# nagyrajmund/st-gcn

Measured on AMD Instinct MI355X. Metric: skeleton clips/sec (fwd+bwd), synthetic (N,3,300,18); 1/2/4/8-GPU scaling, higher is better.
Workload: dtype fp32; 1 GPU; cfg2 Kinetics-skeleton shape: 10-block ST-GCN stack fwd+bwd+CE+Adam, V=18, T=300, K=1 (uni), 400 classes; per_gpu_batch=128, global_batch=128, seq_len=300, parallelism=dp1

## Files before the change

### st-gcn_amd/csrc/internal.h

```cpp
#pragma once
#include <hip/hip_runtime.h>
#include <stdint.h>

#include <type_traits>

namespace stgcn {

struct Dropout {
  uint64_t seed = 0;
  uint32_t thresh = 0;
  float scale = 1.f;
  const uint64_t *seed_dev = nullptr;
};

constexpr uint64_t kDropGolden = 0x9E3779B97F4A7C15ull;

__host__ __device__ inline uint64_t mix64(uint64_t z) {
  z = (z ^ (z >> 30)) * 0xBF58476D1CE4E5B9ull;
  z = (z ^ (z >> 27)) * 0x94D049BB133111EBull;
  return z ^ (z >> 31);
}

__host__ __device__ inline bool dropout_keep(const Dropout &d, uint64_t e) {
  return (uint32_t)(mix64(d.seed + e * kDropGolden) >> 32) >= d.thresh;
// ... 58 lines not shown
  PrevBn prev;
  double *sd, *sdn;
  float *dA;
  float *dA_part;
  int wpk_ready;
  int bna;
  int w4;
};

struct WgradParams {
  const float *P, *Q;
  float *slab;
  int64_t p_bstride, q_bstride;
  int R, C, NQ, s_in, off;
  int M;
  int T_src;
  int V, FT;
  int n_mtiles, n_rtiles, n_jtiles, S, N;
  int CT;
  int bf16;
  int p_bf16, q_bf16;
  int f16x2;
  const unsigned *amax_p, *amax_q;
  BnRef q_bn;
  int x3_mr;
};

hipError_t launch_conv_gemm(const ConvGemmParams &p, hipStream_t s);
hipError_t launch_absmax(const float *x, int64_t n, unsigned *amax, hipStream_t s);
size_t fold_fwd_scratch_floats(int R, int C, int V);
size_t fold_bwd_scratch_floats(int R, int C);
size_t fold_sdz_scratch_doubles(int R, int C, int V);
size_t fold_dwc_floats(int R, int C);
hipError_t launch_fold_w(const float *Wt, const float *W, int R, int C, float *Wc, float *scratch,
                         hipStream_t s);
hipError_t launch_fold_fwd(const float *Wt, const float *W, const float *bt, const float *bZ, int R,
                           int C, int V, int T, int To, int st, float *Wc, double *bq, float *BT,
                           float *scratch, hipStream_t s);
hipError_t launch_fold_prep_bwd(const float *Wt, const float *W, int R, int C, float *scratch,
                                hipStream_t s);
hipError_t launch_fold_tq(const double *cs, int nz, int R, int T, int To, int V, int st,
                          double *Tq, double *tqT, hipStream_t s);
double *fold_sdz_tq_slot(double *scratch, int R, int C);
hipError_t launch_fold_sdz(double *scratch, const float *Wt, const float *Wc, const double *Tq,
                           int R, int C, int V, double *SdZ, double *SdH, hipStream_t s,
                           bool pre = false, const double *tqT = nullptr);
hipError_t launch_fold_small_sd(const double *SdZ, const float *A, const float *bW, int R, int V,
                                float *dbW, float *dA, const double *SdH, int C, double *sd,
                                hipStream_t s);
struct FoldPrepSpec {
  const float *A, *W, *bW, *Wt, *bWt;
  int R, C, V, T, To, stride;
  float *bZ, *Wc, *BT, *fscr_f, *fscr_b;
  double *bq, *f64;
  unsigned *amax;
};
hipError_t launch_fold_prep(const FoldPrepSpec *specs, int n, hipStream_t s);
hipError_t launch_fold_grads(const float *slab, int S, const float *scratch, const float *bZ,
                             const double *Tq, int R, int C, int V, float *dwc, float *dWt,
                             float *dW, hipStream_t s);
struct Bn2Bwd {
  const float *dy = nullptr, *dy_nc = nullptr, *U = nullptr;
  BnRef bn;
  const double *sg = nullptr, *sgu = nullptr;
  float *dU = nullptr, *dUA = nullptr;
  double *sdu = nullptr, *cs = nullptr;
  int N = 0, C = 0, L = 0, V = 0;
  int training = 1;
  Dropout drop;
  int du_bf16 = 0;
  const float *dy_coef = nullptr;
  unsigned *amax = nullptr, *amaxa = nullptr;
  const float *A = nullptr;
};
int apply_cols_chunks(int N);
hipError_t launch_bn_relu_bwd_reduce(const Bn2Bwd &q, double *sg, double *sgu, hipStream_t s);
hipError_t launch_bn_relu_bwd_apply(const Bn2Bwd &q, hipStream_t s);
hipError_t launch_bn_relu_bwd_apply_cols(const Bn2Bwd &q, hipStream_t s);
hipError_t launch_bn_relu_bwd_apply_fr(const Bn2Bwd &q, hipStream_t s);
bool conv_bf16_supported(const ConvGemmParams &p);
size_t conv_bf16_lds_bytes(const ConvGemmParams &p);
hipError_t launch_conv_bf16(const ConvGemmParams &p, hipStream_t s);
bool conv_x3_supported(const ConvGemmParams &p);
constexpr int kPackJobs = 16;
struct PackJob {
  const float *w;
  void *wpk;
  int R, C, NQ, TG, nch, rows, npl;
  int64_t w_sr, w_sc, w_sq, total;
  const unsigned *amax_w;
};
PackJob conv_x3_pack_job(const ConvGemmParams &p, int npl);
size_t conv_x3_pack_bytes(const ConvGemmParams &p, int npl);
hipError_t launch_pack_jobs(const PackJob *jobs, int n, hipStream_t s);
bool conv_x3_bna_supported(const ConvGemmParams &p);
size_t conv_x3_wpk_bytes(const ConvGemmParams &p);
hipError_t launch_conv_x3(const ConvGemmParams &p, hipStream_t s);
bool conv_b1_supported(const ConvGemmParams &p);
hipError_t launch_conv_b1(const ConvGemmParams &p, hipStream_t s);
bool plan_wgrad_x3(WgradParams &w, bool f16x2);
hipError_t launch_wgrad_x3(const WgradParams &p, hipStream_t s);
bool plan_wgrad_bf16(WgradParams &w);
hipError_t launch_wgrad_bf16(const WgradParams &p, hipStream_t s);
hipError_t launch_wgrad(const WgradParams &p, hipStream_t s);
void plan_wgrad_sp(WgradParams &p);
bool wgrad_sp_applies(const WgradParams &p);
inline int wgrad_sp_kc(int CT) { return CT == 64 ? 64 : 32; }
hipError_t launch_wgrad_taps(const WgradParams &p, hipStream_t s);
int wgrad_taps_cb(const WgradParams &p);
size_t wgrad_taps_lds_bytes(const WgradParams &p);
bool wgrad_taps_supported(const WgradParams &p);
size_t conv_gemm_lds_bytes(const ConvGemmParams &p);
size_t conv_gemm_wpk_floats(const ConvGemmParams &p);
bool conv_gemm_supported(const ConvGemmParams &p);
size_t wgrad_lds_bytes(const WgradParams &p);
bool wgrad_supported(const WgradParams &p);
int wgrad_ntiles_j(int C, int NQ);

hipError_t launch_slab_reduce(const float *slab, int S, int64_t n, float *dst, int mode,
                              int R, int K, int C, hipStream_t s);

hipError_t launch_bn_stats(const float *x, int N, int C, int L, double *sum, double *sq,
                           hipStream_t s, unsigned *amax = nullptr);
hipError_t launch_bn_finalize(const double *sum, const double *sq, int C, int64_t M,
                              float eps, float momentum, int training, float *rm, float *rv,
                              float *mean_out, float *invstd_out, hipStream_t s, unsigned *zw = nullptr,
                              int nzw = 0);
hipError_t launch_bn_relu_fwd(const float *U, const BnRef &bn, float *y, int N, int C, int L,
                              double *ysum, double *ysq, Dropout drop, hipStream_t s,
                              double *yext = nullptr, unsigned *ymax = nullptr);
hipError_t launch_chain_coef(const double *sd, const double *sdn, const BnRef &bn1,
                             const double *s1, const double *s2, const double *xst, int C,
                             int64_t M, float *dg1, float *db1, float *coef, double *psum,
                             hipStream_t s);
hipError_t launch_bn_grads_out(const double *sg, const double *sgu, const double *sdu, int C,
                               float *dgamma, float *dbeta, float *dbias, hipStream_t s);
hipError_t launch_bn1_bwd_apply(float *dx, const float *x, const BnRef &bn1, const double *sd,
                                const double *sdn, const float *add, int N, int C, int L,
                                int64_t M, int training, const BnRef &pbn2, double *psum,
                                const float *pU, hipStream_t s);
hipError_t launch_relu_bwd(const float *dy, const float *y, float *dout, double *sum, int N,
                           int C, int L, float scale, hipStream_t s);

hipError_t launch_pack_w(const float *W, float *Wpk, int K, int R, int C, hipStream_t s);
hipError_t launch_bias_rv(const float *A, const float *bW, float *bias_rv, int K, int R, int V,
                          hipStream_t s);
hipError_t launch_bn_finalize_parts(const double *part, int ntiles, int C, int64_t M, float eps,
                                    float momentum, int training, float *rm, float *rv,
                                    float *mean_out, float *invstd_out, hipStream_t s,
                                    double *ys_zero = nullptr, int nw = 0);
template <class F>
inline auto dispatch_v(int V, F &&f) {
  if (V == 18) return f(std::integral_constant<int, 18>{});
  if (V == 25) return f(std::integral_constant<int, 25>{});
  return f(std::integral_constant<int, 50>{});
}

struct SpatialFwd {
  const float *x = nullptr;
  BnRef bn;
  const float *A = nullptr;
  int N = 0, C = 0, R = 0, T = 0, V = 0, K = 0, relu = 0;
  PrevBn prev;
  float *G = nullptr;
  unsigned *amax = nullptr;
  const float *W = nullptr, *biasZ = nullptr;
  void *wpk = nullptr;
// ... 46 lines not shown
```

### st-gcn_amd/csrc/kernels_fold.hip

```cpp
#include <hip/hip_runtime.h>

#include <algorithm>
#include <initializer_list>
#include <vector>

#include "device_common.h"
#include "internal.h"

#define HIP_RET(expr)                  \
  do {                                 \
    hipError_t e_ = (expr);            \
    if (e_ != hipSuccess) return e_;   \
  } while (0)

namespace stgcn {

typedef float float8v __attribute__((ext_vector_type(8)));
typedef double double4v __attribute__((ext_vector_type(4)));

__host__ __device__ inline int pad32(int x) { return (x + 31) & ~31; }

struct FoldJob {
  const float *A, *B;
  int64_t aq, am, bq, bn;
  const double *A2;
  const float *B2;
  int64_t a2q, a2m, b2n;
  void *out;
  int64_t oq, om, on;
  int o_dbl, red;
  int M, N, K, K2;
};

constexpr int kFoldJobs = 18;
struct FoldJobs {
  FoldJob j[kFoldJobs];
  int n;
  int tile0[kFoldJobs + 1];
};

template <int NG>
__device__ __forceinline__ void f32_stream(const float *pa, const float *pb, floatx4 &acc) {
  constexpr int D = NG < 4 ? NG : 4;
  float4 a[D], b[D];
#pragma unroll
  for (int d = 0; d < D; ++d) {
    a[d] = *reinterpret_cast<const float4 *>(pa + 16 * d);
    b[d] = *reinterpret_cast<const float4 *>(pb + 16 * d);
  }
  __builtin_amdgcn_sched_barrier(0);
#pragma unroll
  for (int i = 0; i < NG; ++i) {
    const int d = i % D;
    acc = __builtin_amdgcn_mfma_f32_16x16x4f32(a[d].x, b[d].x, acc, 0, 0, 0);
    acc = __builtin_amdgcn_mfma_f32_16x16x4f32(a[d].y, b[d].y, acc, 0, 0, 0);
    acc = __builtin_amdgcn_mfma_f32_16x16x4f32(a[d].z, b[d].z, acc, 0, 0, 0);
    acc = __builtin_amdgcn_mfma_f32_16x16x4f32(a[d].w, b[d].w, acc, 0, 0, 0);
    if (i + D < NG) {
      a[d] = *reinterpret_cast<const float4 *>(pa + 16 * (i + D));
      b[d] = *reinterpret_cast<const float4 *>(pb + 16 * (i + D));
    }
    __builtin_amdgcn_sched_barrier(0);
  }
}

__device__ __forceinline__ void f32_stream_any(const float *pa, const float *pb, int ng,
                                               floatx4 &acc) {
  switch (ng) {
    case 4: f32_stream<4>(pa, pb, acc); return;
    case 8: f32_stream<8>(pa, pb, acc); return;
    case 16: f32_stream<16>(pa, pb, acc); return;
    default: break;
  }
  for (int i = 0; i < ng; i += 4) {
    if (ng - i >= 4) {
      f32_stream<4>(pa + 16 * i, pb + 16 * i, acc);
    } else {
      for (int k = i; k < ng; ++k) f32_stream<1>(pa + 16 * k, pb + 16 * k, acc);
    }
  }
}

__global__ __launch_bounds__(576) void k_fold_gemm(FoldJobs js) {
  __shared__ float red[9][16 * 17];
  const int tile = blockIdx.x;
  int ji = 0;
  while (ji + 1 < js.n && tile >= js.tile0[ji + 1]) ++ji;
  const FoldJob &g = js.j[ji];
  const int t = tile - js.tile0[ji], ntn = (g.N + 15) >> 4;
  const int m0 = (t / ntn) * 16, n0 = (t % ntn) * 16;
  const int q = threadIdx.x >> 6, l = threadIdx.x & 63, r16 = l & 15, kq = l >> 4;
  floatx4 acc = {0.f, 0.f, 0.f, 0.f};
  {
    const float *pa = g.A + q * g.aq + (int64_t)(m0 + r16) * g.am + 4 * kq;
    const float *pb = g.B + q * g.bq + (int64_t)(n0 + r16) * g.bn + 4 * kq;
    f32_stream_any(pa, pb, (g.K + 15) >> 4, acc);
  }
  if (g.A2) {
    const int m = m0 + r16, n = n0 + r16;
    const bool ok_m = m < g.M, ok_n = n < g.N;
    const double *a2 = g.A2 + q * g.a2q + (int64_t)min(m, g.M - 1) * g.a2m;
    const float *b2 = g.B2 + (int64_t)min(n, g.N - 1) * g.b2n;
    for (int k0 = 0; k0 < g.K2; k0 += 4) {
      const int k = k0 + kq, kc = min(k, g.K2 - 1);
      const float x = (float)a2[kc], y = b2[kc];
      acc = __builtin_amdgcn_mfma_f32_16x16x4f32(k < g.K2 && ok_m ? x : 0.f,
                                                 k < g.K2 && ok_n ? y : 0.f, acc, 0, 0, 0);
    }
  }
  if (!g.red) {
    const int nn = n0 + r16;
#pragma unroll
    for (int r = 0; r < 4; ++r) {
      const int mm = m0 + 4 * kq + r;
      if (mm >= g.M || nn >= g.N) continue;
      const int64_t o = q * g.oq + mm * g.om + nn * g.on;
      if (g.o_dbl)
        reinterpret_cast<double *>(g.out)[o] = acc[r];
      else
        reinterpret_cast<float *>(g.out)[o] = acc[r];
    }
    return;
  }
#pragma unroll
  for (int r = 0; r < 4; ++r) red[q][(4 * kq + r) * 17 + r16] = acc[r];
  __syncthreads();
  if (threadIdx.x >= 256) return;
  const int rr = threadIdx.x >> 4, cc = threadIdx.x & 15;
  const int mm = m0 + rr, nn = n0 + cc;
  if (mm >= g.M || nn >= g.N) return;
  double sum = 0.0;
#pragma unroll
  for (int w = 0; w < 9; ++w) sum += red[w][rr * 17 + cc];
  const int64_t o = mm * g.om + nn * g.on;
  if (g.o_dbl)
    reinterpret_cast<double *>(g.out)[o] = sum;
  else
    reinterpret_cast<float *>(g.out)[o] = (float)sum;
}

static hipError_t fold_gemm_v(const FoldJob *jobs, int n, hipStream_t s) {
  for (int i0 = 0; i0 < n; i0 += kFoldJobs) {
    FoldJobs js{};
    js.n = 0;
    int tiles = 0;
    for (int i = i0; i < std::min(n, i0 + kFoldJobs); ++i) {
      const FoldJob &g = jobs[i];
      if (g.M <= 0 || g.N <= 0) return hipErrorInvalidValue;
      js.j[js.n] = g;
      js.tile0[js.n++] = tiles;
      tiles += ((g.M + 15) / 16) * ((g.N + 15) / 16);
    }
    js.tile0[js.n] = tiles;
    hipLaunchKernelGGL(k_fold_gemm, dim3(tiles), dim3(576), 0, s, js);
  }
  return hipGetLastError();
}

static hipError_t fold_gemm(std::initializer_list<FoldJob> jobs, hipStream_t s) {
  return fold_gemm_v(jobs.begin(), (int)jobs.size(), s);
}

struct TrJob {
  const void *src;
  int s_dbl, S, nq, q_inner;
  int64_t sstride, sq, so, si;
  int O, I;
  void *outQ, *outT;
  int o_dbl;
  int tiles_i;
};

constexpr int kTrJobs = 16;
struct TrJobs {
  TrJob j[kTrJobs];
  int n;
  int tile0[kTrJobs + 1];
};

__global__ __launch_bounds__(576) void k_fold_tr(TrJobs js) {
  __shared__ double tile[36 * 16 + 4];
  const int blk = blockIdx.x, tid = threadIdx.x;
  int ji = 0;
  while (ji + 1 < js.n && blk >= js.tile0[ji + 1]) ++ji;
  const TrJob &g = js.j[ji];
  const int t = blk - js.tile0[ji];
  const int nq = g.nq, OT = nq == 9 ? 4 : 36;
  const int o0 = (t / g.tiles_i) * OT, i0 = (t % g.tiles_i) * 16;
  const int Op = pad32(g.O), Ip = pad32(g.I);
  int oo, ii, q;
  if (nq == 1) {
    oo = tid >> 4; ii = tid & 15; q = 0;
  } else if (g.q_inner) {
    oo = tid / 144; const int r = tid - oo * 144; ii = r / 9; q = r - ii * 9;
  } else {
    oo = tid / 144; const int r = tid - oo * 144; q = r >> 4; ii = r & 15;
  }
  const int o = o0 + oo, i = i0 + ii;
  double v = 0.0;
  if (o < g.O && i < g.I) {
    const int64_t at = q * g.sq + o * g.so + i * g.si;
    if (g.s_dbl) {
      v = reinterpret_cast<const double *>(g.src)[at];
    } else {
      const float *p = reinterpret_cast<const float *>(g.src) + at;
      int k = 0;
      for (; k + 16 <= g.S; k += 16) {
        float a[16];
#pragma unroll
        for (int u = 0; u < 16; ++u) a[u] = p[(int64_t)(k + u) * g.sstride];
#pragma unroll
        for (int u = 0; u < 16; ++u) v += a[u];
      }
      for (; k + 4 <= g.S; k += 4) {
        const float a0 = p[k * g.sstride], a1 = p[(k + 1) * g.sstride],
                    a2 = p[(k + 2) * g.sstride], a3 = p[(k + 3) * g.sstride];
        v += a0;
        v += a1;
        v += a2;
        v += a3;
      }
      for (; k < g.S; ++k) v += p[k * g.sstride];
    }
  }
  const int slot = (q * OT + oo) * 16 + ii;
  tile[slot + slot / 16 / 8] = v;
  __syncthreads();
  if (g.outQ) {
    const int sq2 = tid / (OT * 16), a = (tid >> 4) % OT, b = tid & 15;
    const int s2 = (sq2 * OT + a) * 16 + b;
    const int64_t at = ((int64_t)sq2 * Op + o0 + a) * Ip + i0 + b;
    if (o0 + a < Op) {
      if (g.o_dbl)
        reinterpret_cast<double *>(g.outQ)[at] = tile[s2 + s2 / 16 / 8];
      else
        reinterpret_cast<float *>(g.outQ)[at] = (float)tile[s2 + s2 / 16 / 8];
    }
  }
  if (g.outT) {
    const int sq2 = tid / (OT * 16), a = (tid / OT) & 15, b = tid % OT;
    const int s2 = (sq2 * OT + b) * 16 + a;
    const int64_t at = ((int64_t)sq2 * Ip + i0 + a) * Op + o0 + b;
    if (o0 + b < Op) {
      if (g.o_dbl)
        reinterpret_cast<double *>(g.outT)[at] = tile[s2 + s2 / 16 / 8];
      else
        reinterpret_cast<float *>(g.outT)[at] = (float)tile[s2 + s2 / 16 / 8];
    }
  }
}

static TrJob tr_job(const void *src, int s_dbl, int S, int64_t sstride, int nq, int64_t sq,
                    int64_t so, int64_t si, int O, int I, float *outQ, float *outT,
                    double *outQd = nullptr, double *outTd = nullptr) {
  TrJob g{};
  g.src = src; g.s_dbl = s_dbl; g.S = S; g.sstride = sstride;
  g.nq = nq; g.sq = sq; g.so = so; g.si = si; g.q_inner = sq == 1;
  g.O = O; g.I = I; g.outQ = outQ; g.outT = outT;
  if (outQd || outTd) {
    g.o_dbl = 1;
    g.outQ = outQd;
    g.outT = outTd;
  }
  g.tiles_i = pad32(I) / 16;
  return g;
}

static hipError_t fold_tr_v(const TrJob *jobs, int n, hipStream_t s) {
  for (int i0 = 0; i0 < n; i0 += kTrJobs) {
    TrJobs js{};
    int tiles = 0;
    for (int i = i0; i < std::min(n, i0 + kTrJobs); ++i) {
      const TrJob &g = jobs[i];
      if ((g.nq != 1 && g.nq != 9) || g.O <= 0 || g.I <= 0) return hipErrorInvalidValue;
      js.j[js.n] = g;
      js.tile0[js.n++] = tiles;
      const int OT = g.nq == 9 ? 4 : 36;
      tiles += g.tiles_i * ((pad32(g.O) + OT - 1) / OT);
    }
    js.tile0[js.n] = tiles;
    hipLaunchKernelGGL(k_fold_tr, dim3(tiles), dim3(576), 0, s, js);
  }
  return hipGetLastError();
}

static hipError_t fold_tr(std::initializer_list<TrJob> jobs, hipStream_t s) {
  return fold_tr_v(jobs.begin(), (int)jobs.size(), s);
}

size_t fold_fwd_scratch_floats(int R, int C, int V) {
  const int Rp = pad32(R);
  return (size_t)Rp * (9 * Rp + pad32(C) + pad32(V));
}

static hipError_t fold_fwd_gemms(const float *Wt, const float *W, const float *bZ, int R, int C,
                                 int V, float *Wc, double *bq, float *scratch, hipStream_t s) {
  const int Rp = pad32(R), Cp = pad32(C);
  float *wtq = scratch, *wT = wtq + (size_t)9 * Rp * Rp, *bzT = wT + (size_t)Cp * Rp;
  const TrJob ja = tr_job(Wt, 0, 1, 0, 9, 1, (int64_t)R * 9, 9, R, R, wtq, nullptr);
  const TrJob jb = tr_job(W, 0, 1, 0, 1, 0, C, 1, R, C, nullptr, wT);
  if (bq)
    HIP_RET(fold_tr({ja, jb, tr_job(bZ, 0, 1, 0, 1, 0, V, 1, R, V, nullptr, bzT)}, s));
  else
    HIP_RET(fold_tr({ja, jb}, s));
  FoldJob w{};
  w.A = wtq; w.aq = (int64_t)Rp * Rp; w.am = Rp;
  w.B = wT; w.bn = Rp;
  w.out = Wc; w.oq = 1; w.om = (int64_t)C * 9; w.on = 9;
  w.M = R; w.N = C; w.K = R;
  if (!bq) return fold_gemm({w}, s);
  FoldJob b{};
  b.A = wtq; b.aq = (int64_t)Rp * Rp; b.am = Rp;
  b.B = bzT; b.bn = Rp;
  b.out = bq; b.o_dbl = 1; b.oq = (int64_t)R * V; b.om = V; b.on = 1;
  b.M = R; b.N = V; b.K = R;
  return fold_gemm({w, b}, s);
}

hipError_t launch_fold_w(const float *Wt, const float *W, int R, int C, float *Wc, float *scratch,
                         hipStream_t s) {
  return fold_fwd_gemms(Wt, W, nullptr, R, C, 0, Wc, nullptr, scratch, s);
}

__device__ __forceinline__ int fold_slot_frame(int slot, int nb0, int tb1) {
  return slot < nb0 ? slot : tb1 + slot - nb0;
}

__global__ __launch_bounds__(256) void k_fold_bias(const double *bq, const float *bt, int R, int V,
                                                   int T, int To, int st, float *BT) {
  __shared__ double bs[9 * 256], full[256];
  const int o = blockIdx.x, tid = threadIdx.x;
  for (int e = tid; e < 9 * V; e += 256) {
    const int q = e / V, v = e - q * V;
    bs[e] = bq[((int64_t)q * R + o) * V + v];
  }
  __syncthreads();
  const double b0 = bt[o];
  if (tid < V) {
    double a = b0;
#pragma unroll
    for (int q = 0; q < 9; ++q) a += bs[q * V + tid];
    full[tid] = a;
  }
  __syncthreads();
  float *dst = BT + (int64_t)o * To * V;
  for (int tv = tid; tv < To * V; tv += 256) {
    const int t = tv / V, v = tv - t * V, t0 = st * t - 4;
    double a;
    if (t0 >= 0 && t0 + 8 < T) {
      a = full[v];
    } else {
      a = b0;
      for (int q = 0; q < 9; ++q)
        if (t0 + q >= 0 && t0 + q < T) a += bs[q * V + v];
    }
    dst[tv] = (float)a;
  }
}

static hipError_t fold_bias_frames(const double *bq, const float *bt, int R, int V, int T, int To,
                                   int st, float *BT, hipStream_t s) {
  if (V > 256) return hipErrorInvalidValue;
  hipLaunchKernelGGL(k_fold_bias, dim3(R), dim3(256), 0, s, bq, bt, R, V, T, To, st, BT);
  return hipGetLastError();
}

hipError_t launch_fold_fwd(const float *Wt, const float *W, const float *bt, const float *bZ, int R,
                           int C, int V, int T, int To, int st, float *Wc, double *bq, float *BT,
                           float *scratch, hipStream_t s) {
  HIP_RET(fold_fwd_gemms(Wt, W, bZ, R, C, V, Wc, bq, scratch, s));
  return fold_bias_frames(bq, bt, R, V, T, To, st, BT, s);
}


constexpr int kTqThreads = 1024;
__global__ __launch_bounds__(kTqThreads) void k_fold_tq(const double *cs, int nz, int R, int V,
                                                        int T, int To, int st, int nb0, int tb1,
                                                        double *Tq, double *tqT) {
  __shared__ double ts[kTqThreads], bs[8 * 256];
  const int o = blockIdx.x, tid = threadIdx.x;
  const int Rp = pad32(R), Vp = pad32(V);
  if (o >= R) {
    for (int e = tid; e < 9 * Vp; e += kTqThreads) tqT[(int64_t)e * Rp + o] = 0.0;
    return;
  }
  const int PH = kTqThreads / V, ph = tid / V, v = tid - ph * V;
  const int nsl = nb0 + (To - tb1);
  const int64_t zs = (int64_t)R * To * V;
  double a = 0.0;
  if (ph < PH) {
    const int nj = nz * To;
    auto at = [&](int j) {
      const int z = j / To, t = j - z * To;
      return cs[z * zs + ((int64_t)o * To + t) * V + v];
    };
    double a0 = 0.0, a1 = 0.0, a2 = 0.0, a3 = 0.0;
    int j = ph;
    for (; j + 3 * PH < nj; j += 4 * PH) {
      const double x0 = at(j), x1 = at(j + PH), x2 = at(j + 2 * PH), x3 = at(j + 3 * PH);
      a0 += x0;
      a1 += x1;
      a2 += x2;
      a3 += x3;
    }
    for (; j < nj; j += PH) a0 += at(j);
    a = (a0 + a1) + (a2 + a3);
    for (int sl = ph; sl < nsl; sl += PH) {
      const int t = fold_slot_frame(sl, nb0, tb1);
      double b = 0.0;
      for (int z = 0; z < nz; ++z) b += cs[z * zs + ((int64_t)o * To + t) * V + v];
      bs[sl * V + v] = b;
    }
  }
  ts[tid] = a;
  __syncthreads();
  if (tqT && tid >= V && tid < Vp)
    for (int q = 0; q < 9; ++q) tqT[((int64_t)q * Vp + tid) * Rp + o] = 0.0;
  if (tid >= V) return;
  double tot = 0.0;
  for (int p = 0; p < PH; ++p) tot += ts[p * V + tid];
  for (int q = 0; q < 9; ++q) {
    double r = tot;
    for (int sl = 0; sl < nsl; ++sl) {
      const int tt = st * fold_slot_frame(sl, nb0, tb1) + q - 4;
      if (tt < 0 || tt >= T) r -= bs[sl * V + tid];
    }
    Tq[((int64_t)q * R + o) * V + tid] = r;
    if (tqT) tqT[((int64_t)q * Vp + tid) * Rp + o] = r;
  }
}

void fold_slots(int T, int To, int st, int &nb0, int &tb1) {
  nb0 = std::min(To, (4 + st - 1) / st);
  tb1 = std::max(nb0, std::min(To, (T - 4 + st - 1) / st));
}

hipError_t launch_fold_tq(const double *cs, int nz, int R, int T, int To, int V, int st,
                          double *Tq, double *tqT, hipStream_t s) {
  if (V > 256) return hipErrorInvalidValue;
  int nb0, tb1;
// ... 163 lines not shown
  } else if (Wc) {
    HIP_RET(fold_tr({jt, tr_job(Wc, 0, 1, 0, 9, 1, (int64_t)C * 9, 9, R, C, nullptr, nullptr,
                                nullptr, wcT)},
                    s));
  } else {
    HIP_RET(fold_tr({jt}, s));
  }
  Red64Jobs js{};
  Red64Job z{};
  z.A = wtT; z.aq = (int64_t)Rp * Rp; z.am = Rp;
  z.B = tqT; z.bq = (int64_t)Vp * Rp; z.bn = Rp;
  z.out = SdZ; z.om = V;
  z.M = R; z.N = V; z.K = R;
  js.j[0] = z;
  js.n = 1;
  const int tz = ((R + 15) / 16) * ((V + 15) / 16);
  js.tile0[1] = tz;
  int tiles = tz;
  if (Wc && SdH) {
    Red64Job h = z;
    h.A = wcT; h.aq = (int64_t)Cp * Rp;
    h.out = SdH;
    h.M = C;
    js.j[1] = h;
    js.n = 2;
    tiles += ((C + 15) / 16) * ((V + 15) / 16);
  }
  js.tile0[js.n] = tiles;
  hipLaunchKernelGGL(k_fold_red64, dim3(tiles), dim3(576), 0, s, js);
  return hipGetLastError();
}

__global__ __launch_bounds__(256) void k_fold_small_sd(const double *SdZ, const float *A,
                                                       const float *bW, int R, int V, float *dbW,
                                                       float *dA, const double *SdH, int C,
                                                       double *sd) {
  __shared__ double rs[256], part[256];
  const int tid = threadIdx.x;
  for (int v = tid; v < V; v += 256) {
    double ra = 0.0;
    for (int w = 0; w < V; ++w) ra += (double)A[v * V + w];
    rs[v] = ra;
  }
  __syncthreads();
  if (blockIdx.x > 0) {
    const int c = (blockIdx.x - 1) * blockDim.x + tid;
    if (c >= C) return;
    double a = 0.0;
    for (int v = 0; v < V; ++v) a += SdH[(int64_t)c * V + v] * rs[v];
    sd[c] = a;
    return;
  }
  for (int co = tid; co < R; co += 256) {
    double acc = 0.0;
    for (int v = 0; v < V; ++v) acc += SdZ[co * V + v] * rs[v];
    dbW[co] = (float)acc;
  }
  const int P = 256 / V;
  const int v = tid % V, j = tid / V;
  double acc = 0.0;
  if (j < P)
    for (int co = j; co < R; co += P) acc += (double)bW[co] * SdZ[co * V + v];
  part[tid] = acc;
  __syncthreads();
  if (tid < V) {
    double t = 0.0;
    for (int jj = 0; jj < P; ++jj) t += part[jj * V + tid];
    rs[tid] = t;
  }
  __syncthreads();
  for (int i = tid; i < V * V; i += 256) dA[i] = (float)rs[i / V];
}

hipError_t launch_fold_small_sd(const double *SdZ, const float *A, const float *bW, int R, int V,
                                float *dbW, float *dA, const double *SdH, int C, double *sd,
                                hipStream_t s) {
  if (V > 128) return hipErrorInvalidValue;
  hipLaunchKernelGGL(k_fold_small_sd, dim3(1 + (C + 255) / 256), dim3(256), 0, s, SdZ, A, bW, R, V,
                     dbW, dA, SdH, C, sd);
  return hipGetLastError();
}


constexpr int kPrepJobs = 16;

struct BiasRvJob {
  const float *A, *bW;
  float *out;
  int R, V, blk0;
};
struct BiasRvJobs {
  BiasRvJob j[kPrepJobs];
  int n, blk1;
};

__global__ void k_bias_rv_multi(BiasRvJobs js) {
  int k = 0;
  while (k + 1 < js.n && (int)blockIdx.x >= js.j[k + 1].blk0) ++k;
  const BiasRvJob &q = js.j[k];
  const int idx = ((int)blockIdx.x - q.blk0) * blockDim.x + threadIdx.x;
  if (idx >= q.R * q.V) return;
  const int co = idx / q.V, v = idx - co * q.V;
  double ra = 0.0;
  for (int w = 0; w < q.V; ++w) ra += q.A[(int64_t)v * q.V + w];
  q.out[idx] = (float)((double)q.bW[co] * ra);
}

struct BiasJob {
  const double *bq;
  const float *bt;
  float *BT;
  int R, V, T, To, st, blk0;
};
struct BiasJobs {
  BiasJob j[kPrepJobs];
  int n;
};

__global__ __launch_bounds__(256) void k_fold_bias_multi(BiasJobs js) {
  int k = 0;
  while (k + 1 < js.n && (int)blockIdx.x >= js.j[k + 1].blk0) ++k;
  const BiasJob &q = js.j[k];
  __shared__ double bs[9 * 256], full[256];
  const int o = (int)blockIdx.x - q.blk0, tid = threadIdx.x, V = q.V, R = q.R;
  for (int e = tid; e < 9 * V; e += 256) {
    const int qq = e / V, v = e - qq * V;
    bs[e] = q.bq[((int64_t)qq * R + o) * V + v];
  }
  __syncthreads();
  const double b0 = q.bt[o];
  if (tid < V) {
    double a = b0;
#pragma unroll
    for (int qq = 0; qq < 9; ++qq) a += bs[qq * V + tid];
    full[tid] = a;
  }
  __syncthreads();
  float *dst = q.BT + (int64_t)o * q.To * V;
  for (int tv = tid; tv < q.To * V; tv += 256) {
    const int t = tv / V, v = tv - t * V, t0 = q.st * t - 4;
    double a;
    if (t0 >= 0 && t0 + 8 < q.T) {
      a = full[v];
    } else {
      a = b0;
      for (int qq = 0; qq < 9; ++qq)
        if (t0 + qq >= 0 && t0 + qq < q.T) a += bs[qq * V + v];
    }
    dst[tv] = (float)a;
  }
}

struct AmaxJob {
  const float *x;
  int64_t n;
  unsigned *amax;
};
struct AmaxJobs {
  AmaxJob j[kPrepJobs];
  int n;
};

__global__ __launch_bounds__(256) void k_absmax_multi(AmaxJobs js) {
  const AmaxJob &q = js.j[blockIdx.y];
  float m = 0.f;
  for (int64_t i = (int64_t)blockIdx.x * 256 + threadIdx.x; i < q.n; i += (int64_t)gridDim.x * 256)
    m = fmaxf(m, fabsf(q.x[i]));
  __shared__ float wmax[4];
#pragma unroll
  for (int o = 32; o > 0; o >>= 1) m = fmaxf(m, __shfl_xor(m, o, 64));
  if ((threadIdx.x & 63) == 0) wmax[threadIdx.x >> 6] = m;
  __syncthreads();
  if (threadIdx.x == 0)
    q.amax[blockIdx.x * kAmaxStride] =
        __builtin_bit_cast(unsigned, fmaxf(fmaxf(wmax[0], wmax[1]), fmaxf(wmax[2], wmax[3])));
}

hipError_t launch_fold_prep(const FoldPrepSpec *sp, int n, hipStream_t s) {
  for (int i = 0; i < n; ++i)
    if (sp[i].V > 256 || sp[i].V <= 0 || sp[i].R <= 0 || sp[i].C <= 0) return hipErrorInvalidValue;
  for (int i0 = 0; i0 < n; i0 += kPrepJobs) {
    BiasRvJobs js{};
    int blk = 0;
    for (int i = i0; i < std::min(n, i0 + kPrepJobs); ++i) {
      js.j[js.n] = {sp[i].A, sp[i].bW, sp[i].bZ, sp[i].R, sp[i].V, blk};
      blk += (sp[i].R * sp[i].V + 255) / 256;
      ++js.n;
    }
    js.blk1 = blk;
    hipLaunchKernelGGL(k_bias_rv_multi, dim3(blk), dim3(256), 0, s, js);
  }
  std::vector<TrJob> tr;
  std::vector<FoldJob> fg;
  for (int i = 0; i < n; ++i) {
    const FoldPrepSpec &b = sp[i];
    const int R = b.R, C = b.C, V = b.V, Rp = pad32(R), Cp = pad32(C);
    float *wtq = b.fscr_f, *wT = wtq + (size_t)9 * Rp * Rp, *bzT = wT + (size_t)Cp * Rp;
    tr.push_back(tr_job(b.Wt, 0, 1, 0, 9, 1, (int64_t)R * 9, 9, R, R, wtq, nullptr));
    tr.push_back(tr_job(b.W, 0, 1, 0, 1, 0, C, 1, R, C, nullptr, wT));
    tr.push_back(tr_job(b.bZ, 0, 1, 0, 1, 0, V, 1, R, V, nullptr, bzT));
    float *wtT = b.fscr_b, *wd = wtT + (size_t)9 * Rp * Rp;
    tr.push_back(tr_job(b.Wt, 0, 1, 0, 9, 1, (int64_t)R * 9, 9, R, R, nullptr, wtT));
    tr.push_back(tr_job(b.W, 0, 1, 0, 1, 0, C, 1, R, C, wd, nullptr));
    tr.push_back(tr_job(b.Wt, 0, 1, 0, 9, 1, (int64_t)R * 9, 9, R, R, nullptr, nullptr, nullptr,
                        b.f64));
    FoldJob w{};
    w.A = wtq; w.aq = (int64_t)Rp * Rp; w.am = Rp;
    w.B = wT; w.bn = Rp;
    w.out = b.Wc; w.oq = 1; w.om = (int64_t)C * 9; w.on = 9;
    w.M = R; w.N = C; w.K = R;
    FoldJob q{};
    q.A = wtq; q.aq = (int64_t)Rp * Rp; q.am = Rp;
    q.B = bzT; q.bn = Rp;
    q.out = b.bq; q.o_dbl = 1; q.oq = (int64_t)R * V; q.om = V; q.on = 1;
    q.M = R; q.N = V; q.K = R;
    fg.push_back(w);
    fg.push_back(q);
  }
  HIP_RET(fold_tr_v(tr.data(), (int)tr.size(), s));
  HIP_RET(fold_gemm_v(fg.data(), (int)fg.size(), s));
  for (int i0 = 0; i0 < n; i0 += kPrepJobs) {
    BiasJobs js{};
    AmaxJobs am{};
    int blk = 0;
    for (int i = i0; i < std::min(n, i0 + kPrepJobs); ++i) {
      js.j[js.n++] = {sp[i].bq, sp[i].bWt, sp[i].BT, sp[i].R, sp[i].V, sp[i].T, sp[i].To,
                      sp[i].stride, blk};
      blk += sp[i].R;
      am.j[am.n++] = {sp[i].Wc, (int64_t)sp[i].R * sp[i].C * 9, sp[i].amax};
    }
    hipLaunchKernelGGL(k_fold_bias_multi, dim3(blk), dim3(256), 0, s, js);
    hipLaunchKernelGGL(k_absmax_multi, dim3(kAmaxSlots, am.n), dim3(256), 0, s, am);
  }
  tr.clear();
  for (int i = 0; i < n; ++i) {
    const FoldPrepSpec &b = sp[i];
    const int R = b.R, C = b.C, Rp = pad32(R);
    tr.push_back(tr_job(b.Wc, 0, 1, 0, 9, 1, (int64_t)C * 9, 9, R, C, nullptr, nullptr, nullptr,
                        b.f64 + (size_t)9 * Rp * Rp));
  }
  HIP_RET(fold_tr_v(tr.data(), (int)tr.size(), s));
  return hipGetLastError();
}

}
```

### st-gcn_amd/csrc/kernels_x3.hip

```cpp
#include <hip/hip_runtime.h>

#include <algorithm>
#include <cstdlib>

#include "device_common.h"
#include "internal.h"

constexpr int kWgWriteStart = 1;

namespace stgcn {

typedef float f2v __attribute__((ext_vector_type(2)));
template <int NPL>
__device__ __forceinline__ floatx16 mfma_p(bf16x8 a, bf16x8 b, floatx16 c) {
  if constexpr (NPL == 2)
    return mfma_h(a, b, c);
  else
    return mfma_bf16(a, b, c);
}

__device__ __forceinline__ int f16x2_se(const unsigned *amax) {
  const int e = (int)((amax ? amax_read(amax) : 0x3f800000u) >> 23) & 0xff;
  const int se = e == 0 ? 0 : 140 - e;
  return se < -100 ? -100 : (se > 100 ? 100 : se);
// ... 836 lines not shown
    return;
  }
  if (p.s_out == 1) {
    __syncthreads();
#pragma unroll
    for (int rb = 0; rb < MR; ++rb)
#pragma unroll
      for (int j = 0; j < 2; ++j)
        acc_to_img(smem, acc[rb * 2 + j], mi * 32 * MR + rb * 32, (nj0 + j) * 32);
    __syncthreads();
    if constexpr (BNA) {
      bna_contract<G::ROWS>(smem, arow);
      __syncthreads();
    }
    conv_tile_store_rows<V, G::NCOLS, G::NT, G::ROWS, NPL == 1, NPL != 1>(
        p, smem, smem + G::ROWS * kEpiPitch, n, r0, m0);
    return;
  }
  if constexpr (MR == 1) {
    float *ho = smem + 1024 + (wave & 3) * 2 * 64 * 16;
    __syncthreads();
    if (half == 1) {
#pragma unroll
      for (int j = 0; j < 2; ++j)
#pragma unroll
        for (int i = 0; i < 16; ++i) ho[(j * 16 + i) * 64 + lane] = acc[j][i];
    }
    __syncthreads();
    if (half == 0) {
#pragma unroll
      for (int j = 0; j < 2; ++j)
#pragma unroll
        for (int i = 0; i < 16; ++i) acc[2 + j][i] = ho[(j * 16 + i) * 64 + lane];
      conv_tile_epilogue<V, G::NCOLS, false, NPL == 1, NPL != 1>(p, acc, n, r0, m0, smem);
    } else if (p.stat_sum) {
      __syncthreads();
    }
  }
}

__global__ void k_pack_conv_w_x3(const float *w, __bf16 *wpk, int R, int C, int NQ, int TG,
                                 int nch, int rows, int npl, int64_t w_sr, int64_t w_sc,
                                 int64_t w_sq, int64_t total, const unsigned *amax_w) {
  const int64_t idx = (int64_t)blockIdx.x * blockDim.x + threadIdx.x;
  const int se = npl == 2 ? f16x2_se_bits(amax_w ? amax_read_wave(amax_w) : 0x3f800000u) : 0;
  if (idx >= total) return;
  const int jj = (int)(idx & 7);
  int64_t t = idx >> 3;
  const int rl = (int)(t % rows);
  t /= rows;
  const int o = (int)(t & 1);
  t >>= 1;
  const int qq = (int)(t % TG);
  t /= TG;
  const int pl = (int)(t % npl);
  t /= npl;
  const int NG = NQ / TG;
  const int g = (int)(t % NG);
  t /= NG;
  const int ch = (int)(t % nch);
  const int rt = (int)(t / nch);
  const int r = rt * rows + rl, c = ch * 16 + o * 8 + jj, q = g * TG + qq;
  float v = 0.f;
  if (r < R && c < C) v = w[(int64_t)r * w_sr + (int64_t)c * w_sc + (int64_t)q * w_sq];
  if (npl == 2) {
    const float vs = v * pow2f(se);
    const _Float16 h = (_Float16)vs;
    const _Float16 l = (_Float16)(vs - (float)h);
    reinterpret_cast<_Float16 *>(wpk)[idx] = pl == 0 ? h : l;
    return;
  }
  const __bf16 h = (__bf16)v;
  const float r1 = v - (float)h;
  const __bf16 m = (__bf16)r1;
  const __bf16 l = (__bf16)(r1 - (float)m);
  wpk[idx] = pl == 0 ? h : (pl == 1 ? m : l);
}

struct PackJobs {
  PackJob j[kPackJobs];
  int64_t start[kPackJobs + 1];
  int n;
};

__global__ __launch_bounds__(256) void k_pack_conv_w_x3_multi(PackJobs js) {
  const int64_t gi = (int64_t)blockIdx.x * blockDim.x + threadIdx.x;
  int k = 0;
  while (k + 1 < js.n && gi >= js.start[k + 1]) ++k;
  const PackJob &q = js.j[k];
  const int se = q.npl == 2 ? f16x2_se_bits(q.amax_w ? amax_read_wave(q.amax_w) : 0x3f800000u) : 0;
  const int npl = q.npl, rows = q.rows, TG = q.TG, NG = q.NQ / q.TG;
  const int units = (int)(q.total / (8 * npl));
  const int u0 = (int)(gi - js.start[k]);
  if (u0 >= units) return;
  int t = u0;
  const int rl = t % rows;
  t /= rows;
  const int o = t & 1;
  t >>= 1;
  const int qq = t % TG;
  t /= TG;
  const int g = t % NG;
  t /= NG;
  const int ch = t % q.nch;
  const int rt = t / q.nch;
  const int r = rt * rows + rl, c0 = ch * 16 + o * 8, tap = g * TG + qq;
  float v[8];
  const bool rok = r < q.R;
  const float *src = q.w + (int64_t)(rok ? r : 0) * q.w_sr + (int64_t)tap * q.w_sq;
#pragma unroll
  for (int jj = 0; jj < 8; ++jj)
    v[jj] = (rok && c0 + jj < q.C) ? src[(int64_t)(c0 + jj) * q.w_sc] : 0.f;
  const int64_t base = ((((int64_t)(rt * q.nch + ch) * NG + g) * npl * TG + qq) * 2 + o) *
                           rows * 8 + (int64_t)rl * 8;
  const int64_t pstride = (int64_t)TG * 2 * rows * 8;
  if (npl == 2) {
    const float sc = pow2f(se);
    unsigned hw[4], lw[4];
#pragma unroll
    for (int i = 0; i < 4; ++i) {
      typedef _Float16 h2_t __attribute__((ext_vector_type(2)));
      const float a = v[2 * i] * sc, b = v[2 * i + 1] * sc;
      const _Float16 ha = (_Float16)a, hb = (_Float16)b;
      const h2_t hv = {ha, hb}, lv = {(_Float16)(a - (float)ha), (_Float16)(b - (float)hb)};
      hw[i] = __builtin_bit_cast(unsigned, hv);
      lw[i] = __builtin_bit_cast(unsigned, lv);
    }
    _Float16 *out = reinterpret_cast<_Float16 *>(q.wpk);
    *reinterpret_cast<uint4 *>(out + base) = make_uint4(hw[0], hw[1], hw[2], hw[3]);
    *reinterpret_cast<uint4 *>(out + base + pstride) = make_uint4(lw[0], lw[1], lw[2], lw[3]);
    return;
  }
  __bf16 pv[3][8];
#pragma unroll
  for (int jj = 0; jj < 8; ++jj) {
    const __bf16 h = (__bf16)v[jj];
    const float r1 = v[jj] - (float)h;
    const __bf16 m = (__bf16)r1;
    pv[0][jj] = h;
    pv[1][jj] = m;
    pv[2][jj] = (__bf16)(r1 - (float)m);
  }
  __bf16 *out = reinterpret_cast<__bf16 *>(q.wpk);
#pragma unroll
  for (int pl = 0; pl < 3; ++pl)
    if (pl < npl) {
      unsigned w4[4];
#pragma unroll
      for (int i = 0; i < 4; ++i) {
        const bf16x2 pr = {pv[pl][2 * i], pv[pl][2 * i + 1]};
        w4[i] = __builtin_bit_cast(unsigned, pr);
      }
      *reinterpret_cast<uint4 *>(out + base + pl * pstride) = make_uint4(w4[0], w4[1], w4[2], w4[3]);
    }
}

static int x3_tg(int NQ) { return NQ == 9 ? 3 : NQ; }

bool conv_x3_supported(const ConvGemmParams &p) {
  if (p.C < 16) return false;
  if (p.V != 18 && p.V != 25) return false;
  if (p.FT != kTileCols / p.V) return false;
  if (p.s_in == 2) return p.NQ == 9;
  return p.s_in == 1 && (p.NQ == 9 || p.NQ == 5 || p.NQ == 4);
}

// ... 680 lines not shown
```

Before: 8694 clips/s.

## Merge fold-prep transposes, bias, amax and tail transpose into fewer multi-job kernels

The fold-prep sequence used to issue six transpose jobs per block, then separate bias and absmax kernels, then another transpose launch. It now runs two consolidated kernels: one that writes both transposed outputs (plus an fp64 copy) per source tensor, and a tail kernel that dispatches bias, amax and the Wc transpose by workgroup index. This removes redundant reads of the same weights and several launches on the per-step weight-prep path. Pack job capacity is also doubled so more pack jobs share a single launch. The cost is heavier 576-thread workgroups for the bias and amax parts, where only 256 threads do work.

```diff
diff --git a/st-gcn_amd/csrc/fold_tables.h b/st-gcn_amd/csrc/fold_tables.h
--- /dev/null
+++ b/st-gcn_amd/csrc/fold_tables.h
@@ -0,0 +1,147 @@
+#pragma once
+
+#include <cstddef>
+#include <cstdint>
+
+#if defined(__HIPCC__)
+#define STGCN_HD __host__ __device__
+#else
+#define STGCN_HD
+#endif
+
+namespace stgcn {
+
+STGCN_HD inline int pad32(int x) { return (x + 31) & ~31; }
+
+struct TrJob {
+  const void *src;
+  int s_dbl, S, nq, q_inner;
+  int64_t sstride, sq, so, si;
+  int O, I;
+  void *outQ, *outT;
+  int o_dbl;
+  int tiles_i;
+  double *outT64;
+};
+
+STGCN_HD inline TrJob tr_job(const void *src, int s_dbl, int S, int64_t sstride, int nq,
+                             int64_t sq, int64_t so, int64_t si, int O, int I, float *outQ,
+                             float *outT, double *outQd = nullptr, double *outTd = nullptr) {
+  TrJob g{};
+  g.src = src; g.s_dbl = s_dbl; g.S = S; g.sstride = sstride;
+  g.nq = nq; g.sq = sq; g.so = so; g.si = si; g.q_inner = sq == 1;
+  g.O = O; g.I = I; g.outQ = outQ; g.outT = outT;
+  if (outQd || outTd) {
+    g.o_dbl = 1;
+    g.outQ = outQd;
+    g.outT = outTd;
+  }
+  g.tiles_i = pad32(I) / 16;
+  return g;
+}
+
+STGCN_HD inline int tr_tiles(const TrJob &g) {
+  const int OT = g.nq == 9 ? 4 : 36;
+  return g.tiles_i * ((pad32(g.O) + OT - 1) / OT);
+}
+
+constexpr int kPrepBlocks = 16;
+constexpr int kPrepTrJobs = 3;
+
+struct PrepTrBlock {
+  const float *Wt, *W, *bZ;
+  float *fscr_f, *fscr_b;
+  double *f64;
+  int R, C, V;
+};
+
+struct PrepTrJobs {
+  PrepTrBlock b[kPrepBlocks];
+  int n;
+  int tile0[kPrepBlocks + 1];
+};
+
+STGCN_HD inline TrJob prep_tr_job(const PrepTrBlock &b, int k) {
+  const int R = b.R, C = b.C, V = b.V, Rp = pad32(R), Cp = pad32(C);
+  float *wtq = b.fscr_f, *wT = wtq + (size_t)9 * Rp * Rp, *bzT = wT + (size_t)Cp * Rp;
+  float *wtT = b.fscr_b, *wd = wtT + (size_t)9 * Rp * Rp;
+  switch (k) {
+    case 0: {
+      TrJob g = tr_job(b.Wt, 0, 1, 0, 9, 1, (int64_t)R * 9, 9, R, R, wtq, wtT);
+      g.outT64 = b.f64;
+      return g;
+    }
+    case 1: return tr_job(b.W, 0, 1, 0, 1, 0, C, 1, R, C, wd, wT);
+    default: return tr_job(b.bZ, 0, 1, 0, 1, 0, V, 1, R, V, nullptr, bzT);
+  }
+}
+
+inline int prep_tr_build(PrepTrJobs &js) {
+  int tiles = 0;
+  for (int i = 0; i < js.n; ++i) {
+    js.tile0[i] = tiles;
+    for (int k = 0; k < kPrepTrJobs; ++k) tiles += tr_tiles(prep_tr_job(js.b[i], k));
+  }
+  js.tile0[js.n] = tiles;
+  return tiles;
+}
+
+STGCN_HD inline int prep_tr_find(const PrepTrJobs &js, int tile, int &bi, int &k) {
+  bi = 0;
+  while (bi + 1 < js.n && tile >= js.tile0[bi + 1]) ++bi;
+  int t = tile - js.tile0[bi];
+  for (k = 0; k + 1 < kPrepTrJobs; ++k) {
+    const int nt = tr_tiles(prep_tr_job(js.b[bi], k));
+    if (t < nt) break;
+    t -= nt;
+  }
+  return t;
+}
+
+constexpr int kPrepAmaxSlots = 64;
+enum { PREP_TAIL_BIAS = 0, PREP_TAIL_AMAX = 1, PREP_TAIL_TR = 2 };
+
+struct PrepTailBlock {
+  const double *bq;
+  const float *bt, *Wc;
+  float *BT;
+  unsigned *amax;
+  double *wcT;
+  int R, C, V, T, To, st;
+};
+
+struct PrepTailJobs {
+  PrepTailBlock b[kPrepBlocks];
+  int n;
+  int tile0[kPrepBlocks + 1];
+};
+
+STGCN_HD inline TrJob prep_tail_tr_job(const PrepTailBlock &b) {
+  return tr_job(b.Wc, 0, 1, 0, 9, 1, (int64_t)b.C * 9, 9, b.R, b.C, nullptr, nullptr, nullptr,
+                b.wcT);
+}
+
+inline int prep_tail_build(PrepTailJobs &js) {
+  int tiles = 0;
+  for (int i = 0; i < js.n; ++i) {
+    js.tile0[i] = tiles;
+    tiles += js.b[i].R + kPrepAmaxSlots + tr_tiles(prep_tail_tr_job(js.b[i]));
+  }
+  js.tile0[js.n] = tiles;
+  return tiles;
+}
+
+STGCN_HD inline int prep_tail_find(const PrepTailJobs &js, int tile, int &bi, int &m) {
+  bi = 0;
+  while (bi + 1 < js.n && tile >= js.tile0[bi + 1]) ++bi;
+  int t = tile - js.tile0[bi];
+  m = PREP_TAIL_BIAS;
+  if (t < js.b[bi].R) return t;
+  t -= js.b[bi].R;
+  m = PREP_TAIL_AMAX;
+  if (t < kPrepAmaxSlots) return t;
+  m = PREP_TAIL_TR;
+  return t - kPrepAmaxSlots;
+}
+
+}
diff --git a/st-gcn_amd/csrc/internal.h b/st-gcn_amd/csrc/internal.h
--- a/st-gcn_amd/csrc/internal.h
+++ b/st-gcn_amd/csrc/internal.h
@@ -164,7 +164,7 @@
 size_t conv_bf16_lds_bytes(const ConvGemmParams &p);
 hipError_t launch_conv_bf16(const ConvGemmParams &p, hipStream_t s);
 bool conv_x3_supported(const ConvGemmParams &p);
-constexpr int kPackJobs = 16;
+constexpr int kPackJobs = 32;
 struct PackJob {
   const float *w;
   void *wpk;
diff --git a/st-gcn_amd/csrc/kernels_fold.hip b/st-gcn_amd/csrc/kernels_fold.hip
--- a/st-gcn_amd/csrc/kernels_fold.hip
+++ b/st-gcn_amd/csrc/kernels_fold.hip
@@ -5,6 +5,7 @@
 #include <vector>
 
 #include "device_common.h"
+#include "fold_tables.h"
 #include "internal.h"
 
 #define HIP_RET(expr)                  \
@@ -17,8 +18,6 @@
 
 typedef float float8v __attribute__((ext_vector_type(8)));
 typedef double double4v __attribute__((ext_vector_type(4)));
-
-__host__ __device__ inline int pad32(int x) { return (x + 31) & ~31; }
 
 struct FoldJob {
   const float *A, *B;
@@ -161,30 +160,16 @@
   return fold_gemm_v(jobs.begin(), (int)jobs.size(), s);
 }
 
-struct TrJob {
-  const void *src;
-  int s_dbl, S, nq, q_inner;
-  int64_t sstride, sq, so, si;
-  int O, I;
-  void *outQ, *outT;
-  int o_dbl;
-  int tiles_i;
-};
-
-constexpr int kTrJobs = 16;
+constexpr int kTrJobs = 4;
 struct TrJobs {
   TrJob j[kTrJobs];
   int n;
   int tile0[kTrJobs + 1];
 };
 
-__global__ __launch_bounds__(576) void k_fold_tr(TrJobs js) {
-  __shared__ double tile[36 * 16 + 4];
-  const int blk = blockIdx.x, tid = threadIdx.x;
-  int ji = 0;
-  while (ji + 1 < js.n && blk >= js.tile0[ji + 1]) ++ji;
-  const TrJob &g = js.j[ji];
-  const int t = blk - js.tile0[ji];
+constexpr int kTrTileDoubles = 36 * 16 + 4;
+
+__device__ __forceinline__ void fold_tr_body(const TrJob &g, int t, int tid, double *tile) {
   const int nq = g.nq, OT = nq == 9 ? 4 : 36;
   const int o0 = (t / g.tiles_i) * OT, i0 = (t % g.tiles_i) * 16;
   const int Op = pad32(g.O), Ip = pad32(g.I);
@@ -237,33 +222,28 @@
         reinterpret_cast<float *>(g.outQ)[at] = (float)tile[s2 + s2 / 16 / 8];
     }
   }
-  if (g.outT) {
+  if (g.outT || g.outT64) {
     const int sq2 = tid / (OT * 16), a = (tid / OT) & 15, b = tid % OT;
     const int s2 = (sq2 * OT + b) * 16 + a;
     const int64_t at = ((int64_t)sq2 * Ip + i0 + a) * Op + o0 + b;
     if (o0 + b < Op) {
-      if (g.o_dbl)
-        reinterpret_cast<double *>(g.outT)[at] = tile[s2 + s2 / 16 / 8];
-      else
-        reinterpret_cast<float *>(g.outT)[at] = (float)tile[s2 + s2 / 16 / 8];
-    }
-  }
-}
-
-static TrJob tr_job(const void *src, int s_dbl, int S, int64_t sstride, int nq, int64_t sq,
-                    int64_t so, int64_t si, int O, int I, float *outQ, float *outT,
-                    double *outQd = nullptr, double *outTd = nullptr) {
-  TrJob g{};
-  g.src = src; g.s_dbl = s_dbl; g.S = S; g.sstride = sstride;
-  g.nq = nq; g.sq = sq; g.so = so; g.si = si; g.q_inner = sq == 1;
-  g.O = O; g.I = I; g.outQ = outQ; g.outT = outT;
-  if (outQd || outTd) {
-    g.o_dbl = 1;
-    g.outQ = outQd;
-    g.outT = outTd;
-  }
-  g.tiles_i = pad32(I) / 16;
-  return g;
+      if (g.outT) {
+        if (g.o_dbl)
+          reinterpret_cast<double *>(g.outT)[at] = tile[s2 + s2 / 16 / 8];
+        else
+          reinterpret_cast<float *>(g.outT)[at] = (float)tile[s2 + s2 / 16 / 8];
+      }
+      if (g.outT64) g.outT64[at] = tile[s2 + s2 / 16 / 8];
+    }
+  }
+}
+
+__global__ __launch_bounds__(576) void k_fold_tr(TrJobs js) {
+  __shared__ double tile[kTrTileDoubles];
+  const int blk = blockIdx.x;
+  int ji = 0;
+  while (ji + 1 < js.n && blk >= js.tile0[ji + 1]) ++ji;
+  fold_tr_body(js.j[ji], blk - js.tile0[ji], threadIdx.x, tile);
 }
 
 static hipError_t fold_tr_v(const TrJob *jobs, int n, hipStream_t s) {
@@ -275,8 +255,7 @@
       if ((g.nq != 1 && g.nq != 9) || g.O <= 0 || g.I <= 0) return hipErrorInvalidValue;
       js.j[js.n] = g;
       js.tile0[js.n++] = tiles;
-      const int OT = g.nq == 9 ? 4 : 36;
-      tiles += g.tiles_i * ((pad32(g.O) + OT - 1) / OT);
+      tiles += tr_tiles(g);
     }
     js.tile0[js.n] = tiles;
     hipLaunchKernelGGL(k_fold_tr, dim3(tiles), dim3(576), 0, s, js);
@@ -326,11 +305,12 @@
   return slot < nb0 ? slot : tb1 + slot - nb0;
 }
 
-__global__ __launch_bounds__(256) void k_fold_bias(const double *bq, const float *bt, int R, int V,
-                                                   int T, int To, int st, float *BT) {
-  __shared__ double bs[9 * 256], full[256];
-  const int o = blockIdx.x, tid = threadIdx.x;
-  for (int e = tid; e < 9 * V; e += 256) {
+constexpr int kBiasLdsDoubles = 10 * 256;
+__device__ __forceinline__ void fold_bias_body(const double *bq, const float *bt, int R, int V,
+                                               int T, int To, int st, float *BT, int o, int tid,
+                                               double *bs, double *full) {
+  const bool act = tid < 256;
+  for (int e = act ? tid : 9 * V; e < 9 * V; e += 256) {
     const int q = e / V, v = e - q * V;
     bs[e] = bq[((int64_t)q * R + o) * V + v];
   }
@@ -344,7 +324,7 @@
   }
   __syncthreads();
   float *dst = BT + (int64_t)o * To * V;
-  for (int tv = tid; tv < To * V; tv += 256) {
+  for (int tv = act ? tid : To * V; tv < To * V; tv += 256) {
     const int t = tv / V, v = tv - t * V, t0 = st * t - 4;
     double a;
     if (t0 >= 0 && t0 + 8 < T) {
@@ -356,6 +336,12 @@
     }
     dst[tv] = (float)a;
   }
+}
+
+__global__ __launch_bounds__(256) void k_fold_bias(const double *bq, const float *bt, int R, int V,
+                                                   int T, int To, int st, float *BT) {
+  __shared__ double lds[kBiasLdsDoubles];
+  fold_bias_body(bq, bt, R, V, T, To, st, BT, blockIdx.x, threadIdx.x, lds, lds + 9 * 256);
 }
 
 static hipError_t fold_bias_frames(const double *bq, const float *bt, int R, int V, int T, int To,
@@ -685,15 +671,13 @@
 }
 
 
-constexpr int kPrepJobs = 16;
-
 struct BiasRvJob {
   const float *A, *bW;
   float *out;
   int R, V, blk0;
 };
 struct BiasRvJobs {
-  BiasRvJob j[kPrepJobs];
+  BiasRvJob j[kPrepBlocks];
   int n, blk1;
 };
 
@@ -709,83 +693,55 @@
   q.out[idx] = (float)((double)q.bW[co] * ra);
 }
 
-struct BiasJob {
-  const double *bq;
-  const float *bt;
-  float *BT;
-  int R, V, T, To, st, blk0;
-};
-struct BiasJobs {
-  BiasJob j[kPrepJobs];
-  int n;
-};
-
-__global__ __launch_bounds__(256) void k_fold_bias_multi(BiasJobs js) {
-  int k = 0;
-  while (k + 1 < js.n && (int)blockIdx.x >= js.j[k + 1].blk0) ++k;
-  const BiasJob &q = js.j[k];
-  __shared__ double bs[9 * 256], full[256];
-  const int o = (int)blockIdx.x - q.blk0, tid = threadIdx.x, V = q.V, R = q.R;
-  for (int e = tid; e < 9 * V; e += 256) {
-    const int qq = e / V, v = e - qq * V;
-    bs[e] = q.bq[((int64_t)qq * R + o) * V + v];
-  }
-  __syncthreads();
-  const double b0 = q.bt[o];
-  if (tid < V) {
-    double a = b0;
-#pragma unroll
-    for (int qq = 0; qq < 9; ++qq) a += bs[qq * V + tid];
-    full[tid] = a;
-  }
-  __syncthreads();
-  float *dst = q.BT + (int64_t)o * q.To * V;
-  for (int tv = tid; tv < q.To * V; tv += 256) {
-    const int t = tv / V, v = tv - t * V, t0 = q.st * t - 4;
-    double a;
-    if (t0 >= 0 && t0 + 8 < q.T) {
-      a = full[v];
-    } else {
-      a = b0;
-      for (int qq = 0; qq < 9; ++qq)
-        if (t0 + qq >= 0 && t0 + qq < q.T) a += bs[qq * V + v];
-    }
-    dst[tv] = (float)a;
-  }
-}
-
-struct AmaxJob {
-  const float *x;
-  int64_t n;
-  unsigned *amax;
-};
-struct AmaxJobs {
-  AmaxJob j[kPrepJobs];
-  int n;
-};
-
-__global__ __launch_bounds__(256) void k_absmax_multi(AmaxJobs js) {
-  const AmaxJob &q = js.j[blockIdx.y];
+__global__ __launch_bounds__(576) void k_fold_prep_tr(PrepTrJobs js) {
+  __shared__ double tile[kTrTileDoubles];
+  int bi, k;
+  const int t = prep_tr_find(js, blockIdx.x, bi, k);
+  fold_tr_body(prep_tr_job(js.b[bi], k), t, threadIdx.x, tile);
+}
+
+__device__ __forceinline__ void absmax_slot_body(const float *x, int64_t n, unsigned *amax,
+                                                 int slot, int tid, float *wmax) {
   float m = 0.f;
-  for (int64_t i = (int64_t)blockIdx.x * 256 + threadIdx.x; i < q.n; i += (int64_t)gridDim.x * 256)
-    m = fmaxf(m, fabsf(q.x[i]));
-  __shared__ float wmax[4];
+  if (tid < 256)
+    for (int64_t i = (int64_t)slot * 256 + tid; i < n; i += (int64_t)kAmaxSlots * 256)
+      m = fmaxf(m, fabsf(x[i]));
 #pragma unroll
   for (int o = 32; o > 0; o >>= 1) m = fmaxf(m, __shfl_xor(m, o, 64));
-  if ((threadIdx.x & 63) == 0) wmax[threadIdx.x >> 6] = m;
-  __syncthreads();
-  if (threadIdx.x == 0)
-    q.amax[blockIdx.x * kAmaxStride] =
+  if ((tid & 63) == 0 && tid < 256) wmax[tid >> 6] = m;
+  __syncthreads();
+  if (tid == 0)
+    amax[slot * kAmaxStride] =
         __builtin_bit_cast(unsigned, fmaxf(fmaxf(wmax[0], wmax[1]), fmaxf(wmax[2], wmax[3])));
+}
+
+static_assert(sizeof(PrepTrJobs) <= 4096 && sizeof(PrepTailJobs) <= 4096 &&
+                  sizeof(FoldJobs) <= 4096,
+              "the job tables travel in the kernel arguments");
+static_assert(kPrepAmaxSlots == kAmaxSlots, "fold_tables.h counts one workgroup per amax slot");
+static_assert(kTrTileDoubles <= kBiasLdsDoubles, "the members share the bias member's LDS");
+
+__global__ __launch_bounds__(576) void k_fold_prep_tail(PrepTailJobs js) {
+  __shared__ double lds[kBiasLdsDoubles];
+  int bi, m;
+  const int t = prep_tail_find(js, blockIdx.x, bi, m);
+  const PrepTailBlock &b = js.b[bi];
+  const int tid = threadIdx.x;
+  if (m == PREP_TAIL_BIAS)
+    fold_bias_body(b.bq, b.bt, b.R, b.V, b.T, b.To, b.st, b.BT, t, tid, lds, lds + 9 * 256);
+  else if (m == PREP_TAIL_AMAX)
+    absmax_slot_body(b.Wc, (int64_t)b.R * b.C * 9, b.amax, t, tid, reinterpret_cast<float *>(lds));
+  else
+    fold_tr_body(prep_tail_tr_job(b), t, tid, lds);
 }
 
 hipError_t launch_fold_prep(const FoldPrepSpec *sp, int n, hipStream_t s) {
   for (int i = 0; i < n; ++i)
     if (sp[i].V > 256 || sp[i].V <= 0 || sp[i].R <= 0 || sp[i].C <= 0) return hipErrorInvalidValue;
-  for (int i0 = 0; i0 < n; i0 += kPrepJobs) {
+  for (int i0 = 0; i0 < n; i0 += kPrepBlocks) {
     BiasRvJobs js{};
     int blk = 0;
-    for (int i = i0; i < std::min(n, i0 + kPrepJobs); ++i) {
+    for (int i = i0; i < std::min(n, i0 + kPrepBlocks); ++i) {
       js.j[js.n] = {sp[i].A, sp[i].bW, sp[i].bZ, sp[i].R, sp[i].V, blk};
       blk += (sp[i].R * sp[i].V + 255) / 256;
       ++js.n;
@@ -793,20 +749,20 @@
     js.blk1 = blk;
     hipLaunchKernelGGL(k_bias_rv_multi, dim3(blk), dim3(256), 0, s, js);
   }
-  std::vector<TrJob> tr;
+  for (int i0 = 0; i0 < n; i0 += kPrepBlocks) {
+    PrepTrJobs js{};
+    for (int i = i0; i < std::min(n, i0 + kPrepBlocks); ++i) {
+      const FoldPrepSpec &b = sp[i];
+      js.b[js.n++] = {b.Wt, b.W, b.bZ, b.fscr_f, b.fscr_b, b.f64, b.R, b.C, b.V};
+    }
+    const int tiles = prep_tr_build(js);
+    hipLaunchKernelGGL(k_fold_prep_tr, dim3(tiles), dim3(576), 0, s, js);
+  }
   std::vector<FoldJob> fg;
   for (int i = 0; i < n; ++i) {
     const FoldPrepSpec &b = sp[i];
     const int R = b.R, C = b.C, V = b.V, Rp = pad32(R), Cp = pad32(C);
     float *wtq = b.fscr_f, *wT = wtq + (size_t)9 * Rp * Rp, *bzT = wT + (size_t)Cp * Rp;
-    tr.push_back(tr_job(b.Wt, 0, 1, 0, 9, 1, (int64_t)R * 9, 9, R, R, wtq, nullptr));
-    tr.push_back(tr_job(b.W, 0, 1, 0, 1, 0, C, 1, R, C, nullptr, wT));
-    tr.push_back(tr_job(b.bZ, 0, 1, 0, 1, 0, V, 1, R, V, nullptr, bzT));
-    float *wtT = b.fscr_b, *wd = wtT + (size_t)9 * Rp * Rp;
-    tr.push_back(tr_job(b.Wt, 0, 1, 0, 9, 1, (int64_t)R * 9, 9, R, R, nullptr, wtT));
-    tr.push_back(tr_job(b.W, 0, 1, 0, 1, 0, C, 1, R, C, wd, nullptr));
-    tr.push_back(tr_job(b.Wt, 0, 1, 0, 9, 1, (int64_t)R * 9, 9, R, R, nullptr, nullptr, nullptr,
-                        b.f64));
     FoldJob w{};
     w.A = wtq; w.aq = (int64_t)Rp * Rp; w.am = Rp;
     w.B = wT; w.bn = Rp;
@@ -820,29 +776,17 @@
     fg.push_back(w);
     fg.push_back(q);
   }
-  HIP_RET(fold_tr_v(tr.data(), (int)tr.size(), s));
   HIP_RET(fold_gemm_v(fg.data(), (int)fg.size(), s));
-  for (int i0 = 0; i0 < n; i0 += kPrepJobs) {
-    BiasJobs js{};
-    AmaxJobs am{};
-    int blk = 0;
-    for (int i = i0; i < std::min(n, i0 + kPrepJobs); ++i) {
-      js.j[js.n++] = {sp[i].bq, sp[i].bWt, sp[i].BT, sp[i].R, sp[i].V, sp[i].T, sp[i].To,
-                      sp[i].stride, blk};
-      blk += sp[i].R;
-      am.j[am.n++] = {sp[i].Wc, (int64_t)sp[i].R * sp[i].C * 9, sp[i].amax};
-    }
-    hipLaunchKernelGGL(k_fold_bias_multi, dim3(blk), dim3(256), 0, s, js);
-    hipLaunchKernelGGL(k_absmax_multi, dim3(kAmaxSlots, am.n), dim3(256), 0, s, am);
-  }
-  tr.clear();
-  for (int i = 0; i < n; ++i) {
-    const FoldPrepSpec &b = sp[i];
-    const int R = b.R, C = b.C, Rp = pad32(R);
-    tr.push_back(tr_job(b.Wc, 0, 1, 0, 9, 1, (int64_t)C * 9, 9, R, C, nullptr, nullptr, nullptr,
-                        b.f64 + (size_t)9 * Rp * Rp));
-  }
-  HIP_RET(fold_tr_v(tr.data(), (int)tr.size(), s));
+  for (int i0 = 0; i0 < n; i0 += kPrepBlocks) {
+    PrepTailJobs js{};
+    for (int i = i0; i < std::min(n, i0 + kPrepBlocks); ++i) {
+      const FoldPrepSpec &b = sp[i];
+      js.b[js.n++] = {b.bq, b.bWt, b.Wc, b.BT, b.amax, b.f64 + (size_t)9 * pad32(b.R) * pad32(b.R),
+                      b.R, b.C, b.V, b.T, b.To, b.stride};
+    }
+    const int tiles = prep_tail_build(js);
+    hipLaunchKernelGGL(k_fold_prep_tail, dim3(tiles), dim3(576), 0, s, js);
+  }
   return hipGetLastError();
 }
 
diff --git a/st-gcn_amd/csrc/kernels_x3.hip b/st-gcn_amd/csrc/kernels_x3.hip
--- a/st-gcn_amd/csrc/kernels_x3.hip
+++ b/st-gcn_amd/csrc/kernels_x3.hip
@@ -942,6 +942,7 @@
   int64_t start[kPackJobs + 1];
   int n;
 };
+static_assert(sizeof(PackJobs) <= 4096, "the job table travels in the kernel arguments");
 
 __global__ __launch_bounds__(256) void k_pack_conv_w_x3_multi(PackJobs js) {
   const int64_t gi = (int64_t)blockIdx.x * blockDim.x + threadIdx.x;
```

Measured after the change: 8653 clips/s. No clear change (-0.5%).
